# ielab/llm-rankers

Measured on AMD Instinct MI355X. Metric: passages/sec (pointwise yes_no reranking, flan-t5-large shape), higher is better.
Workload: dtype f16 (MFMA inputs), f32 accumulate + residual stream

## Files before the change

llm-rankers_amd/csrc/rk_engine.hip:

```cpp
#include <hip/hip_runtime.h>
#include <dlfcn.h>
#include <rccl/rccl.h>

#include <algorithm>
#include <cmath>
#include <cstdarg>
#include <cstdio>
#include <cstdlib>
#include <cstring>
#include <map>
#include <atomic>
#include <string>
#include <vector>

#include "../../include/rk_engine.h"
#include "attention.h"
#include "attention_d128.h"
#include "decoder_kernels.h"
#include "gemm.h"
#include "gemv_rows.h"
#include "llama_kernels.h"
#include "llama_kernels_hd64.h"
#include "misc_kernels.h"

// ... 50 lines not shown
template <class T>
struct Grown {
  T* p = nullptr; size_t cap = 0;
  Grown() = default;
  Grown(const Grown&) = delete;
  Grown& operator=(const Grown&) = delete;
  ~Grown() { if (p) hipFree(p); }
  int reserve(rk_engine* e, size_t n, int* gen = nullptr);
};

enum DecBuf { IX_DEC_IDS, IX_OUT_IDS, IX_LAST_ROWS, IX_N_CACHED, IX_ROW_LABEL = IX_N_CACHED, IX_ROW_OFF, IX_OUT_IDX, IX_ROW_SEQ, IX_TREE_KEYS, IX_TREE_POS, IX_COUNT };
struct DecIndex {
  struct Src { DecBuf b; const std::vector<int>& v; };
  int* d[IX_COUNT] = {nullptr};
  int* pin = nullptr;
  static constexpr int PIN_INTS = 8192;
  int put(rk_engine* e, hipStream_t st, DecBuf b, const int* src, int n);
  int write(rk_engine* e, hipStream_t st, std::initializer_list<Src> srcs);
  int tree(rk_engine* e, hipStream_t st, std::vector<int>& sig, std::initializer_list<Src> srcs);
 private:
  std::vector<int> held[IX_N_CACHED], tree_sig;
  unsigned long epoch = 0, tree_epoch = ~0ul;
};

}

#define RK_SLOTS 2

struct Slot {
  hipStream_t se = nullptr, sd = nullptr;
  NormStream enc;
  half_t *qkv = nullptr, *ctx = nullptr, *ffh = nullptr, *enc_out = nullptr;
  int* d_tokens = nullptr; int* d_seq_off = nullptr;
  int n_seq = 0, T = 0, maxL = 0, minL = 0; bool staged = false; int last_floats = 0;
  half_t* cross_kv = nullptr;
  DecIndex idx; int* d_argmax = nullptr;
  NormStream dec;
  half_t *dqkv = nullptr, *dctx = nullptr, *dq = nullptr, *dffh = nullptr, *dlast = nullptr;
  float* dssq_few[2] = {nullptr, nullptr};
  half_t *xqk = nullptr, *xctx = nullptr;
  float *xpart = nullptr, *xstat = nullptr; bool have_cross_kv = false;
  float* d_scores = nullptr; float* h_scores = nullptr;
  hipEvent_t ev_enc = nullptr, ev_dec = nullptr; bool dec_pending = false;
};

struct rk_engine {
  rk_model_desc d{};
  int dev = 0;
  std::string err;
  bool finalized = false;
  int inner = 0;
  std::map<std::string, HostTensor> host;
  std::vector<void*> allocs;
  half_t *emb = nullptr, *lm_head = nullptr, *cross_kv_w = nullptr;
  std::vector<EncLayerW> enc;
  std::vector<DecLayerW> dec;
  float *enc_final_ln = nullptr, *dec_final_ln = nullptr, *lut_enc = nullptr, *lut_dec = nullptr;
  Grown<float> logits;
  Grown<float> amax_val; Grown<int> amax_idx; int amax_gen = 0;
  Grown<half_t> kv_cache; int kv_gen = 0;
  Grown<int> gen_buf; int* gen_pin = nullptr; hipEvent_t ev_gen[2] = {nullptr, nullptr};
  size_t scores_cap = 0;
  Slot slots[RK_SLOTS];
  struct Options {
    int glds = 1, skinny = 0x3F, overlap = 1, gemm_variant = 0, attn_short = 5, xattn_direct = 1, attn_heads_per_wg = 0, attn_ko = 0,
        gemm_persistent = 1, fold_norm = 1, s64_stages = 0, dec_fold_norm = 1, greedy_spec = 160, consumer_stats = 1, xattn_mfma = 1,
        dec_ffn_tiled = 1, gemm_split = 1, dec_fuse = 1, dec_fuse_rows = 0, dec_attn_seq = 1, attn_long = 1, attn_long_nw = 0,
        llama_attn_dma = 1, attn_long_xcd = 1, llama_attn_nw = 0, dec_graph = 1, gemm_sk = 1, dec_cross_mfma = 1, dec_gemv = 1, dec_gemv_rows = 4,
        dec_cached_attn = 1, llama_dec_r = 0;
  } opt;
  float* attn_trace = nullptr;
  int n_cu = 256;
  struct SkWs { hipStream_t st = nullptr; float* slabs = nullptr; int* cnt = nullptr; };
  SkWs sk_ws[2 * RK_SLOTS];
  hipEvent_t t0 = nullptr, t1 = nullptr, t_tmp = nullptr;
  bool prof_on = false;
  std::vector<ProfRec> prof_recs; size_t prof_used = 0;
  double prof_flops[PC_COUNT] = {0}, prof_bytes[PC_COUNT] = {0}; int64_t prof_n[PC_COUNT] = {0};
  int family = 0; rk_llama_desc ld{};
  float rope_factor = 0.f, rope_low = 1.f, rope_high = 4.f; int rope_orig = 0;
  bool qkv_bias = false;
  int window = 0;
  std::vector<LlamaLayerW> ll; float *l_final_ln = nullptr, *rope_cos = nullptr, *rope_sin = nullptr; int* d_pos = nullptr;
  Grown<half_t> lkv; Grown<float> lpart; Grown<int> lints; int lkv_gen = 0;
  struct LlamaStep { NormStream stream; half_t *qkv = nullptr, *ctx = nullptr, *ffh = nullptr; } lg;
  struct LlamaSession {
    bool open = false; int n_slots = 0, max_len = 0, cap = 0, seen = 0;
    std::vector<int> busy, told, len, max_new, col, done;
  } ls;
  struct GraphEntry { int seen = 0; bool failed = false; hipGraphExec_t exec = nullptr; };
  std::map<std::vector<int>, GraphEntry> graphs; int opt_epoch = 0;
  ncclComm_t comm = nullptr; int comm_rank = 0, comm_world = 1;
  float* d_gather[RK_SLOTS] = {nullptr}; float* h_gather[RK_SLOTS] = {nullptr}; size_t gather_cap = 0;
  hipEvent_t ev_gather[RK_SLOTS] = {nullptr}; bool gather_pending[RK_SLOTS] = {false}; int gather_n[RK_SLOTS] = {0};
  float *d_gsend = nullptr, *d_gall = nullptr, *h_gall = nullptr, *h_gstage = nullptr;
  hipEvent_t ev_gall = nullptr, ev_append = nullptr; bool gall_pending = false, append_foreign = false; int gall_n = 0;
};

namespace {

int fail(rk_engine* e, int code, const char* fmt, ...) {
  char buf[1024];
// ... 831 lines not shown
  p.cgrid = dim3(n_heads, rows);
  p.window = e->window;
  return p;
}

void launch_llama_dec_attn(rk_engine* e, hipStream_t st, const LlamaDecAttnPlan& p, LlamaDecAttnArgs a, int rows) {
  a.nch = p.nch; a.window = p.window;
  Bracket br(e, st, PC_DEC_ATTN, 4.0 * rows * (double)a.P * a.n_heads * p.hd, 2.0 * rows * (double)a.P * a.n_kv * p.hd * 2.0);
  with_width(p.hd, [&](auto W) {
    constexpr int D = decltype(W)::value;
    auto go = [&](auto rc) {
      constexpr int R = decltype(rc)::value;
      if constexpr (R == 7 && D != 128) abort();
      else if (p.window > 0) {
        if (a.bias) hipLaunchKernelGGL((attn_dec_cached_win_kernel<D, R, true>), p.grid, dim3(256), 0, st, a);
        else hipLaunchKernelGGL((attn_dec_cached_win_kernel<D, R, false>), p.grid, dim3(256), 0, st, a);
      }
      else if (a.bias) hipLaunchKernelGGL((attn_dec_cached_kernel<D, R, true>), p.grid, dim3(256), 0, st, a);
      else hipLaunchKernelGGL((attn_dec_cached_kernel<D, R, false>), p.grid, dim3(256), 0, st, a);
    };
    using std::integral_constant;
    switch (p.R) {
      case 8: go(integral_constant<int, 8>{}); break;
      case 7: go(integral_constant<int, 7>{}); break;
      case 4: go(integral_constant<int, 4>{}); break;
      case 2: go(integral_constant<int, 2>{}); break;
      default: go(integral_constant<int, 1>{}); break;
    }
    if (p.window > 0) hipLaunchKernelGGL(attn_dec_combine_win_kernel<D>, p.cgrid, dim3(D), 0, st, a);
    else hipLaunchKernelGGL(attn_dec_combine_kernel<D>, p.cgrid, dim3(D), 0, st, a);
  });
}

int run_encoder(rk_engine* e, Slot& sl, bool need_cross_kv) {
  const rk_model_desc& d = e->d;
  hipStream_t st = enc_stream(e, sl);
  const int T = sl.T, I = e->inner, dm = d.d_model, F = d.d_ff;
  const bool own = e->opt.consumer_stats != 0;
  int rc = RK_OK;
  NormStream ns = sl.enc;
  const EncAttnPlan ap = plan_enc_attn(e, sl.n_seq, sl.maxL, sl.minL, d.n_heads);
  ns.begin(e, st, sl.d_tokens, T, e->opt.fold_norm != 0);
  for (int l = 0; l < d.n_enc_layers; ++l) {
    const EncLayerW& w = e->enc[l];
    const bool last = l + 1 == d.n_enc_layers;
    RC(gemm(e, st, ns.consumer(e, st, w.ln0, Gemm(PC_ENC_GEMM_QKV, EPI_STORE_F16, ns.x(), dm, ns.fold ? w.qkv_f : w.qkv, dm, sl.qkv, 3 * I, T, 3 * I, dm), own)));
    launch_enc_attn(e, st, EncAttnCall{sl.qkv, sl.ctx, sl.d_seq_off, e->lut_enc, 3 * I, I, I, d.n_heads, sl.n_seq, sl.maxL, sl.T}, ap);
    RC(ns.producer(e, st, Gemm(PC_ENC_GEMM_O, EPI_RESID_F32, sl.ctx, I, w.o, I, ns.hidden, dm, T, dm, I)));
    RC(gemm(e, st, ns.consumer(e, st, w.ln1, Gemm(PC_ENC_GEMM_FFN_IN, d.gated_gelu ? EPI_GEGLU_F16 : EPI_RELU_F16, ns.x(), dm, ns.fold ? w.ffn_in_f : w.ffn_in, dm,
                                                 sl.ffh, F, T, d.gated_gelu ? 2 * F : F, dm), own)));
    RC(ns.producer(e, st, Gemm(PC_ENC_GEMM_FFN_OUT, EPI_RESID_F32, sl.ffh, F, w.ffn_out, F, ns.hidden, dm, T, dm, F), !last));
  }
  rmsnorm(e, st, ns.hidden, e->enc_final_ln, sl.enc_out, nullptr, T);
  if (need_cross_kv)
    RC(gemm(e, st, Gemm(PC_GEMM_CROSS_KV, EPI_STORE_F16, sl.enc_out, dm, e->cross_kv_w, dm, sl.cross_kv, 2 * I, T, d.n_dec_layers * 2 * I, dm)
                       .split(2 * I, (long)d.max_tokens * 2 * I)));
  sl.have_cross_kv = need_cross_kv;
  HIPCHK(e, hipGetLastError());
  return RK_OK;
}

struct DecRows {
  int rows; const int* keys; const int* pos; const int* seq;
  const int* row_off; int seq0, n_seq; bool cross_kv; const int* ids;
  bool tree() const { return keys != nullptr; }
};
struct DecCache { half_t* kv; int P; const int* pos; const int* tree_keys; int* tree_pos; };
void launch_dec_cached_step(const rk_engine* e, hipStream_t st, const AttnCachedArgs& ca, int B, int H, const int* tree_keys, int* tree_pos) {
  if (e->opt.dec_cached_attn) {
    hipLaunchKernelGGL(attn_dec_cached_kernel, dim3(H, B), dim3(256), attn_dec_lds(ca.P), st, ca);
  } else {
    hipLaunchKernelGGL(kv_append_kernel, dim3(B), dim3(256), 0, st, ca, tree_pos);
    hipLaunchKernelGGL(attn_dec_kernel, dim3(1, H, B), dim3(256), attn_dec_lds(ca.P), st,
                       AttnDecArgs{ca.qkv, ca.ldqkv, ca.cache, ca.cache + ca.inner, 2 * ca.inner, nullptr, ca.ctx, ca.ldctx, ca.bias_lut, ca.P, 1, ca.P,
                                   tree_keys, tree_pos});
  }
}
int run_decoder(rk_engine* e, Slot& sl, int Ld, const DecRows* rows = nullptr, const DecCache* cache = nullptr) {
  const rk_model_desc& d = e->d;
  hipStream_t st = dec_stream(e, sl);
  const bool tree = rows && rows->tree(), ragged = rows && !rows->tree();
  const int B = ragged ? rows->n_seq : sl.n_seq, M = rows ? rows->rows : B * Ld, I = e->inner, dm = d.d_model, F = d.d_ff;
  const bool have_kv = ragged ? rows->cross_kv : sl.have_cross_kv;
  const int* seq_off = sl.d_seq_off + (ragged ? rows->seq0 : 0);
  const DecLenClass lc = dec_len_class(e, Ld);
  if (tree && (have_kv || lc.one)) return fail(e, RK_ERR_STATE, "the tree form needs the query-side cross-attention and L_d >= 2");
  if (ragged && have_kv && !sl.have_cross_kv) return fail(e, RK_ERR_STATE, "the ragged pass needs the K / V the encoder did not materialise");
  if (cache && (rows || have_kv || Ld != 1)) return fail(e, RK_ERR_STATE, "the incremental pass needs the query-side cross-attention and one row per sequence");
  if (wide_heads(e) && (!lc.one || rows || cache || have_kv || e->opt.dec_fuse == 2))
    return refuse_wide(e, "run_decoder", "this pass would launch a 64-wide kernel");
  const bool ws = lc.stream;
  const bool dfold = ws && e->opt.dec_fold_norm && (e->opt.skinny & 0x3F) == 0x3F;
  const bool fuse_asked = e->opt.dec_fuse == 2 || (e->opt.dec_fuse == 1 && lc.one);
  const bool few = dfold && e->opt.dec_gemv && !lc.one && M <= e->opt.dec_gemv_rows && !fuse_asked &&
                   gemv_fits(M, dm) && gemv_fits(M, I) && gemv_fits(M, F);
  const GemmFamily fam = few ? GEMM_GEMV : (ws ? GEMM_STREAM : GEMM_TILED);
  int rc = RK_OK;
  NormStream ns = sl.dec;
  if (few) { ns.ssq[0] = sl.dssq_few[0]; ns.ssq[1] = sl.dssq_few[1]; }
  auto normed = [&](const float* ln, Gemm c) { return ns.consumer(e, st, ln, c.on(fam), true); };
  auto resid = [&](Gemm c, bool stats = true) { return ns.producer(e, st, c.on(fam), stats); };
  ns.begin(e, st, ragged && rows->ids ? rows->ids : sl.idx.d[IX_DEC_IDS], M, dfold);
  const DecAttnPlan self_plan = plan_dec_attn(e, false, B, Ld, Ld, d.n_heads, tree ? rows->rows : 0);
  const DecAttnPlan cross_plan = plan_dec_attn(e, true, B, Ld, sl.maxL, d.n_heads, 0);
  for (int l = 0; l < d.n_dec_layers; ++l) {
    const DecLayerW& w = e->dec[l];
    if (!cache && lc.one) {
      RC(resid(normed(w.ln0, Gemm(PC_DEC_GEMM, EPI_RESID_F32, ns.x(), dm, dfold ? w.ov_f : w.ov, dm, ns.hidden, dm, M, dm, dm))));
    } else {
      RC(gemm(e, st, normed(w.ln0, Gemm(PC_DEC_GEMM, EPI_STORE_F16, ns.x(), dm, dfold ? w.qkv_f : w.qkv, dm, sl.dqkv, 3 * I, M, 3 * I, dm))));
      if (cache) {
        const AttnCachedArgs ca{sl.dqkv, 3 * I, cache->kv + (size_t)l * B * cache->P * 2 * I, cache->P, I, cache->pos, sl.dctx, I, e->lut_dec};
        Bracket br(e, st, PC_DEC_ATTN, 4.0 * B * (double)cache->P * I, (double)B * cache->P * 2 * I * 2.0);
        launch_dec_cached_step(e, st, ca, B, d.n_heads, cache->tree_keys, cache->tree_pos);
      } else {
        launch_dec_attn(e, st, self_plan, AttnDecArgs{sl.dqkv, 3 * I, sl.dqkv + I, sl.dqkv + 2 * I, 3 * I, nullptr, sl.dctx, I, e->lut_dec, Ld, 1, Ld,
                                                      tree ? rows->keys : nullptr, tree ? rows->pos : nullptr, 0, ragged ? rows->row_off : nullptr},
                        4.0 * M * Ld * I, 0);
      }
      RC(resid(Gemm(PC_DEC_GEMM, EPI_RESID_F32, sl.dctx, I, w.o, I, ns.hidden, dm, M, dm, I)));
    }
    const Gemm cq = normed(w.ln1, Gemm(PC_DEC_GEMM, EPI_STORE_F16, ns.x(), dm, dfold ? w.cq_f : w.cq, dm, sl.dq, I, M, I, dm));
    if (!have_kv) {
      RC(run_xattn_chain(e, st, XAttnChain{cq.A, cq.lda, cq.W, w.ckT, e->cross_kv_w + ((size_t)l * 2 * I + I) * dm, cq.fold, cq.family,
                                           sl.enc_out, sl.d_seq_off, rows ? rows->seq : nullptr, Ld, 0, sl.dq, sl.xqk, sl.xpart, sl.xstat, sl.xctx,
                                           sl.dctx, I, M, d.n_heads, dm, sl.maxL, sl.T, fuse_asked, head_width(e)}));
    } else {
      RC(gemm(e, st, cq));
      const half_t* kv = sl.cross_kv + (size_t)l * d.max_tokens * 2 * I;
      launch_dec_attn(e, st, cross_plan, AttnDecArgs{sl.dq, I, kv, kv + I, 2 * I, seq_off, sl.dctx, I, nullptr, Ld, 0, sl.maxL, nullptr, nullptr, 0,
                                                       ragged ? rows->row_off : nullptr},
                      4.0 * Ld * (double)sl.T * I, (double)sl.T * 2 * I * 2.0);
    }
    RC(resid(Gemm(PC_DEC_GEMM, EPI_RESID_F32, sl.dctx, I, w.co, I, ns.hidden, dm, M, dm, I)));
    {
      const bool tiled_in = dfold && e->opt.dec_ffn_tiled && lc.one;
      RC(gemm(e, st, ns.consumer(e, st, w.ln2, Gemm(PC_DEC_GEMM, d.gated_gelu ? EPI_GEGLU_F16 : EPI_RELU_F16, ns.x(), dm, dfold ? w.ffn_in_f : w.ffn_in, dm,
                                                   sl.dffh, F, M, d.gated_gelu ? 2 * F : F, dm).on(tiled_in ? GEMM_TILED : fam), true)));
    }
    RC(resid(Gemm(PC_DEC_GEMM, EPI_RESID_F32, sl.dffh, F, w.ffn_out, F, ns.hidden, dm, M, dm, F), l + 1 < d.n_dec_layers));
  }
  HIPCHK(e, hipGetLastError());
  return RK_OK;
}

int encoder_then_handoff_kv(rk_engine* e, Slot& sl, bool need_cross_kv) {
  hipStream_t se = enc_stream(e, sl), sd = dec_stream(e, sl);
  if (need_cross_kv && !sl.cross_kv) return refuse_wide(e, "encoder", "the materialised cross-attention K / V are not allocated");
  if (sl.dec_pending && sd != se) HIPCHK(e, hipStreamWaitEvent(se, sl.ev_dec, 0));
  int rc = run_encoder(e, sl, need_cross_kv);
  if (rc) return rc;
  if (sd != se) {
    HIPCHK(e, hipEventRecord(sl.ev_enc, se));
    HIPCHK(e, hipStreamWaitEvent(sd, sl.ev_enc, 0));
  }
  return RK_OK;
}

int encoder_then_handoff(rk_engine* e, Slot& sl, int max_ld, bool query_side = false) {
  return encoder_then_handoff_kv(e, sl, !query_side && !use_xattn_direct(e, sl, max_ld));
}

int mark_decoder_done(rk_engine* e, Slot& sl) {
  HIPCHK(e, hipEventRecord(sl.ev_dec, dec_stream(e, sl)));
  sl.dec_pending = true;
  return RK_OK;
}

int sync_all(rk_engine* e) {
  for (Slot& sl : e->slots) {
    HIPCHK(e, hipStreamSynchronize(sl.se));
    HIPCHK(e, hipStreamSynchronize(sl.sd));
  }
  return RK_OK;
}

int finish_blocking(rk_engine* e, Slot& sl) {
  int rc = mark_decoder_done(e, sl);
  if (rc || (rc = sync_all(e))) return rc;
  sl.dec_pending = false;
  return RK_OK;
}

template <class T>
int Grown<T>::reserve(rk_engine* e, size_t n, int* gen) {
  if (n <= cap) return RK_OK;
  int rc = sync_all(e);
  if (rc) return rc;
// ... 44 lines not shown
int put_dec_ids_shared(rk_engine* e, Slot& sl, const int32_t* prefix, int Ld) {
  std::vector<int> ids((size_t)sl.n_seq * Ld);
  for (int b = 0; b < sl.n_seq; ++b) memcpy(&ids[(size_t)b * Ld], prefix, Ld * sizeof(int));
  return sl.idx.put(e, dec_stream(e, sl), IX_DEC_IDS, ids.data(), (int)ids.size());
}

void shift_right(const int32_t* labels, int n, std::vector<int>* out) {
  for (int t = 0; t < n; ++t) out->push_back(t ? labels[t - 1] : 0);
}

int check_greedy_args(rk_engine* e, const int32_t* dec_prefix, int dec_len, int max_new) {
  if (!dec_prefix || dec_len <= 0 || max_new <= 0 || dec_len + max_new - 1 > e->d.max_dec_len)
    return fail(e, RK_ERR_CAPACITY, "dec_len %d + max_new %d exceeds max_dec_len %d", dec_len, max_new, e->d.max_dec_len);
  return RK_OK;
}

int read_scores_blocking(rk_engine* e, Slot& sl, hipStream_t st, size_t n, float* out) {
  HIPCHK(e, hipMemcpyAsync(sl.h_scores, sl.d_scores, n * sizeof(float), hipMemcpyDeviceToHost, st));
  if (e->family == 0) { const int rc = finish_blocking(e, sl); if (rc) return rc; }
  else HIPCHK(e, hipStreamSynchronize(st));
  HIPCHK(e, hipGetLastError());
  memcpy(out, sl.h_scores, n * sizeof(float));
  return RK_OK;
}

int stage_slot(rk_engine* e, int slot, const int32_t* tokens, const int32_t* seq_offsets, int n_seq) {
  if (slot < 0 || slot >= RK_SLOTS) return fail(e, RK_ERR_INVALID, "slot %d out of range", slot);
  if (e->family != 0) return fail(e, RK_ERR_STATE, "T5 entry point called on a Llama engine (use rk_llama_*)");
  int rc = set_device(e);
  if (rc) return rc;
  Slot& sl = e->slots[slot];
  sl.staged = false;
  if ((rc = check_batch(e, &sl, tokens, seq_offsets, n_seq))) return rc;
  if (sl.dec_pending) { HIPCHK(e, hipEventSynchronize(sl.ev_dec)); sl.dec_pending = false; }
  HIPCHK(e, hipStreamSynchronize(enc_stream(e, sl)));
  HIPCHK(e, hipMemcpy(sl.d_tokens, tokens, (size_t)sl.T * sizeof(int), hipMemcpyHostToDevice));
  HIPCHK(e, hipMemcpy(sl.d_seq_off, seq_offsets, (size_t)(n_seq + 1) * sizeof(int), hipMemcpyHostToDevice));
  sl.staged = true;
  return RK_OK;
}

enum GraphKind { GK_T5_SCORE, GK_T5_GREEDY_STEP, GK_T5_GREEDY2, GK_T5_GENERATE_STEP, GK_LLAMA_STEP, GK_T5_COMPARE, GK_LLAMA_SESSION_STEP };
template <class F>
int run_graphed(rk_engine* e, hipStream_t st, std::vector<int> key, F&& body) {
  key.push_back(e->opt_epoch);
  if (!e->opt.dec_graph || e->prof_on) return body();
  auto& g = e->graphs[key];
  if (g.exec) { HIPCHK(e, hipGraphLaunch(g.exec, st)); return RK_OK; }
  if (g.failed || g.seen++ == 0) return body();
  if (e->graphs.size() > 256) {
    for (auto& kv : e->graphs) if (kv.second.exec && &kv.second != &g) { hipGraphExecDestroy(kv.second.exec); kv.second.exec = nullptr; kv.second.seen = 0; }
  }
  hipGraph_t graph = nullptr;
  if (hipStreamBeginCapture(st, hipStreamCaptureModeThreadLocal) != hipSuccess) { (void)hipGetLastError(); g.failed = true; return body(); }
  const int rc = body();
  const hipError_t ec = hipStreamEndCapture(st, &graph);
  if (rc != RK_OK || ec != hipSuccess || !graph) {
    (void)hipGetLastError();
    if (graph) hipGraphDestroy(graph);
    g.failed = true;
    return rc != RK_OK ? rc : body();
  }
  const hipError_t ei = hipGraphInstantiate(&g.exec, graph, nullptr, nullptr, 0);
  hipGraphDestroy(graph);
  if (ei != hipSuccess || !g.exec) { (void)hipGetLastError(); g.exec = nullptr; g.failed = true; return body(); }
  HIPCHK(e, hipGraphLaunch(g.exec, st));
  return RK_OK;
}

int ensure_decode_ring(rk_engine* e) {
// ... 210 lines not shown
  const rk_model_desc& d = *desc;
  if (d.d_kv != 64 && d.d_kv != 128)
    return fail(nullptr, RK_ERR_INVALID, "d_kv=%d unsupported: the gfx950 attention kernels are built for d_kv=64 and, for one decoder position, d_kv=128", d.d_kv);
  if (d.d_model % 64 || (d.n_heads * d.d_kv) % 64 || d.d_ff % 64 || d.vocab % 4)
    return fail(nullptr, RK_ERR_INVALID, "d_model, n_heads*d_kv, d_ff must be multiples of 64 and vocab of 4");
  if (d.d_model > 4096)
    return fail(nullptr, RK_ERR_INVALID, "d_model=%d unsupported: rmsnorm_kernel holds a row of at most 4096 columns in registers (d_model <= 4096)", d.d_model);
  if (d.max_distance > RK_LUT_R || d.n_buckets < 4 || d.n_buckets > 256)
    return fail(nullptr, RK_ERR_INVALID, "relative attention config unsupported (max_distance<=%d)", RK_LUT_R);
  if (d.max_tokens <= 0 || d.max_seqs <= 0 || d.max_dec_len <= 0 || d.n_enc_layers <= 0 || d.n_dec_layers <= 0)
    return fail(nullptr, RK_ERR_INVALID, "capacities and layer counts must be positive");
  if ((long)d.max_seqs * d.max_dec_len > 8192 * 8) return fail(nullptr, RK_ERR_INVALID, "max_seqs*max_dec_len too large");
  int n_dev = 0;
  if (hipGetDeviceCount(&n_dev) != hipSuccess || n_dev <= 0)
    return fail(nullptr, RK_ERR_NO_DEVICE, "no HIP device visible: this engine has no CPU path");
  if (device_ordinal < 0 || device_ordinal >= n_dev)
    return fail(nullptr, RK_ERR_NO_DEVICE, "device ordinal %d out of range (%d devices)", device_ordinal, n_dev);
  hipDeviceProp_t prop;
  if (hipGetDeviceProperties(&prop, device_ordinal) != hipSuccess)
    return fail(nullptr, RK_ERR_HIP, "hipGetDeviceProperties failed");
  if (strncmp(prop.gcnArchName, "gfx950", 6) != 0)
    return fail(nullptr, RK_ERR_NO_DEVICE, "device %d is %s; kernels are built for gfx950 (MI355X) only", device_ordinal, prop.gcnArchName);
  rk_engine* e = new rk_engine();
  e->d = d; e->dev = device_ordinal; e->n_cu = prop.multiProcessorCount > 0 ? prop.multiProcessorCount : 256; e->inner = d.n_heads * d.d_kv;
  int prio_lo = 0, prio_hi = 0;
  bool ok = hipSetDevice(device_ordinal) == hipSuccess;
  ok = ok && hipDeviceGetStreamPriorityRange(&prio_lo, &prio_hi) == hipSuccess;
  for (int i = 0; ok && i < RK_SLOTS; ++i)
    ok = hipStreamCreateWithPriority(&e->slots[i].se, hipStreamNonBlocking, prio_lo) == hipSuccess &&
         hipStreamCreateWithPriority(&e->slots[i].sd, hipStreamNonBlocking, prio_hi) == hipSuccess;
  ok = ok && hipEventCreate(&e->t0) == hipSuccess && hipEventCreate(&e->t1) == hipSuccess &&
       hipEventCreateWithFlags(&e->t_tmp, hipEventDisableTiming) == hipSuccess;
  for (int i = 0; ok && i < RK_SLOTS; ++i)
    ok = hipEventCreateWithFlags(&e->slots[i].ev_enc, hipEventDisableTiming) == hipSuccess &&
         hipEventCreateWithFlags(&e->slots[i].ev_dec, hipEventDisableTiming) == hipSuccess;
  for (int i = 0; ok && i < 2 * RK_SLOTS; ++i) {
    rk_engine::SkWs& w = e->sk_ws[i];
    w.st = (i & 1) ? e->slots[i >> 1].sd : e->slots[i >> 1].se;
    ok = hipMalloc((void**)&w.slabs, (size_t)KSPLIT_MAX_SLABS * 65536 * sizeof(float)) == hipSuccess &&
         hipMalloc((void**)&w.cnt, KSPLIT_MAX_SLABS * sizeof(int)) == hipSuccess &&
         hipMemset(w.cnt, 0, KSPLIT_MAX_SLABS * sizeof(int)) == hipSuccess;
  }
  if (!ok) {
    for (auto& w : e->sk_ws) { if (w.slabs) hipFree(w.slabs); if (w.cnt) hipFree(w.cnt); }
    delete e;
    return fail(nullptr, RK_ERR_HIP, "stream/event/workspace creation failed");
  }
  *out = e;
  return RK_OK;
}

void rk_engine_destroy(rk_engine* e) {
  if (!e) return;
  hipSetDevice(e->dev);
  for (auto& sl : e->slots) {
    if (sl.se) hipStreamSynchronize(sl.se);
    if (sl.sd) hipStreamSynchronize(sl.sd);
  }
  comm_release(e);
  for (auto& kv : e->graphs) if (kv.second.exec) hipGraphExecDestroy(kv.second.exec);
  e->graphs.clear();
  for (void* p : e->allocs) hipFree(p);
  if (e->gen_pin) hipHostFree(e->gen_pin);
  for (hipEvent_t ev : e->ev_gen) if (ev) hipEventDestroy(ev);
  for (auto& w : e->sk_ws) { if (w.slabs) hipFree(w.slabs); if (w.cnt) hipFree(w.cnt); }
  for (auto& sl : e->slots) {
    if (sl.h_scores) hipHostFree(sl.h_scores);
    if (sl.idx.pin) hipHostFree(sl.idx.pin);
    if (sl.ev_enc) hipEventDestroy(sl.ev_enc);
    if (sl.ev_dec) hipEventDestroy(sl.ev_dec);
  }
  for (auto& r : e->prof_recs) { hipEventDestroy(r.a); hipEventDestroy(r.b); }
  if (e->t0) hipEventDestroy(e->t0);
  if (e->t1) hipEventDestroy(e->t1);
  if (e->t_tmp) hipEventDestroy(e->t_tmp);
  for (auto& sl : e->slots) {
    if (sl.se) hipStreamDestroy(sl.se);
    if (sl.sd) hipStreamDestroy(sl.sd);
  }
  delete e;
}

int rk_engine_load_tensor(rk_engine* e, const char* hf_name, const void* data, int dtype, const int64_t* shape, int ndim) {
  if (!e || !hf_name || !data || !shape) return fail(e, RK_ERR_INVALID, "null argument");
  if (e->finalized) return fail(e, RK_ERR_STATE, "engine already finalized");
  if (ndim < 1 || ndim > 2) return RK_OK;
  std::string name(hf_name);
  if (name == "encoder.embed_tokens.weight" || name == "decoder.embed_tokens.weight") return RK_OK;
  size_t n = 1;
  for (int i = 0; i < ndim; ++i) n *= (size_t)shape[i];
  HostTensor t;
  t.shape.assign(shape, shape + ndim);
  const bool keep_f32 = ndim == 1 || name.find("relative_attention_bias") != std::string::npos;
  auto get = [&](size_t i) -> float {
    switch (dtype) {
      case RK_F32: return ((const float*)data)[i];
      case RK_F16: return (float)((const half_t*)data)[i];
      case RK_BF16: { uint32_t u = (uint32_t)((const uint16_t*)data)[i] << 16; float f; memcpy(&f, &u, 4); return f; }
      default: return 0.f;
    }
  };
  if (dtype < RK_F32 || dtype > RK_BF16) return fail(e, RK_ERR_INVALID, "unknown dtype %d", dtype);
// ... 125 lines not shown
  RC(up_h(&e->cross_kv_w, ckv));
  {
    half_t* d_vT = nullptr; float* d_ov32 = nullptr;
    RC(dalloc(e, &d_vT, (size_t)dm * I)); RC(dalloc(e, &d_ov32, (size_t)dm * dm));
    std::vector<half_t> vT((size_t)dm * I), ov16((size_t)dm * dm);
    std::vector<float> ov32((size_t)dm * dm);
    for (int l = 0; l < d.n_dec_layers; ++l) {
      const std::string p = "decoder.block." + std::to_string(l) + ".layer.0.SelfAttention.";
      const auto& wv = H(p + "v.weight");
      for (int j = 0; j < I; ++j)
        for (int k = 0; k < dm; ++k) vT[(size_t)k * I + j] = wv[(size_t)j * dm + k];
      HIPCHK(e, hipMemcpy(d_vT, vT.data(), vT.size() * 2, hipMemcpyHostToDevice));
      RC(gemm(e, e->slots[0].se, Gemm(PC_OTHER, EPI_STORE_F32, e->dec[l].o, I, d_vT, I, d_ov32, dm, dm, dm, I)));
      HIPCHK(e, hipStreamSynchronize(e->slots[0].se));
      HIPCHK(e, hipMemcpy(ov32.data(), d_ov32, ov32.size() * 4, hipMemcpyDeviceToHost));
      for (size_t i = 0; i < ov32.size(); ++i) ov16[i] = (half_t)ov32[i];
      RC(up_h(&e->dec[l].ov, ov16));
      const auto& ln0 = Fv("decoder.block." + std::to_string(l) + ".layer.0.layer_norm.weight");
      for (size_t i = 0; i < ov32.size(); ++i) ov16[i] = (half_t)(ov32[i] * ln0[i % dm]);
      RC(up_h(&e->dec[l].ov_f, ov16));
    }
    HIPCHK(e, hipGetLastError());
  }
  e->host.clear();

  const size_t Tc = d.max_tokens, Bc = d.max_seqs, Mc = (size_t)d.max_seqs * d.max_dec_len;
  e->scores_cap = Bc * 64;
  if (2 * e->scores_cap < 7 * Bc) return fail(e, RK_ERR_CAPACITY, "score buffer of %zu floats cannot hold a compare of %zu sequences", e->scores_cap, Bc);
  for (Slot& sl : e->slots) {
    RC(dalloc(e, &sl.enc.hidden, Tc * dm)); RC(dalloc(e, &sl.enc.xn, Tc * dm)); RC(dalloc(e, &sl.qkv, Tc * 3 * I));
    RC(dalloc(e, &sl.ctx, Tc * I)); RC(dalloc(e, &sl.ffh, Tc * F)); RC(dalloc(e, &sl.enc_out, Tc * dm));
    RC(dalloc(e, &sl.enc.xraw[0], Tc * dm)); RC(dalloc(e, &sl.enc.ssq[0], Tc * ((dm + 63) / 64))); RC(dalloc(e, &sl.enc.factors, Tc + 512));
    HIPCHK(e, hipMemset(sl.enc.factors, 0, (Tc + 512) * sizeof(float)));
    RC(dalloc(e, &sl.d_tokens, Tc)); RC(dalloc(e, &sl.d_seq_off, Bc + 1));
    if (!wide_heads(e)) RC(dalloc(e, &sl.cross_kv, (size_t)d.n_dec_layers * Tc * 2 * I));
    RC(dalloc(e, &sl.idx.d[IX_DEC_IDS], Mc)); RC(dalloc(e, &sl.idx.d[IX_LAST_ROWS], Bc)); RC(dalloc(e, &sl.idx.d[IX_OUT_IDS], 8192));
    RC(dalloc(e, &sl.idx.d[IX_ROW_LABEL], Mc)); RC(dalloc(e, &sl.idx.d[IX_ROW_OFF], 2 * Bc + 1)); RC(dalloc(e, &sl.idx.d[IX_OUT_IDX], Bc)); RC(dalloc(e, &sl.d_argmax, Bc));
    RC(dalloc(e, &sl.idx.d[IX_ROW_SEQ], Mc)); RC(dalloc(e, &sl.idx.d[IX_TREE_KEYS], Mc * (size_t)d.max_dec_len)); RC(dalloc(e, &sl.idx.d[IX_TREE_POS], Mc));
    RC(dalloc(e, &sl.dec.hidden, Mc * dm)); RC(dalloc(e, &sl.dec.xn, Mc * dm)); RC(dalloc(e, &sl.dqkv, Mc * 3 * I));
    RC(dalloc(e, &sl.dctx, Mc * I)); RC(dalloc(e, &sl.dq, Mc * I)); RC(dalloc(e, &sl.dffh, Mc * F));
    RC(dalloc(e, &sl.dlast, Bc * dm));
    for (int i = 0; i < 2; ++i) { RC(dalloc(e, &sl.dec.xraw[i], Mc * dm)); RC(dalloc(e, &sl.dec.ssq[i], Mc * ((dm + 31) / 32))); RC(dalloc(e, &sl.dssq_few[i], (size_t)GEMV_MAX_ROWS * e->n_cu)); }
    RC(dalloc(e, &sl.dec.factors, Mc));
    RC(dalloc(e, &sl.xqk, (size_t)XA_MAX_ROWS * d.n_heads * dm)); RC(dalloc(e, &sl.xctx, (size_t)XA_MAX_ROWS * d.n_heads * dm));
    RC(dalloc(e, &sl.xpart, (size_t)XA_MAX_CHUNKS * d.n_heads * dm)); RC(dalloc(e, &sl.xstat, (size_t)XA_MAX_CHUNKS * d.n_heads * 2));
    RC(dalloc(e, &sl.d_scores, e->scores_cap));
    HIPCHK(e, hipHostMalloc((void**)&sl.h_scores, e->scores_cap * sizeof(float), hipHostMallocDefault));
    HIPCHK(e, hipHostMalloc((void**)&sl.idx.pin, IX_N_CACHED * DecIndex::PIN_INTS * sizeof(int), hipHostMallocDefault));
  }
  const int dec_smem_max = (int)attn_dec_lds(std::max(d.max_tokens, d.max_dec_len));
  (void)hipFuncSetAttribute((const void*)attn_dec_kernel, hipFuncAttributeMaxDynamicSharedMemorySize, std::min(dec_smem_max, 160 * 1024));
  (void)hipFuncSetAttribute((const void*)attn_dec_seq_kernel, hipFuncAttributeMaxDynamicSharedMemorySize, 160 * 1024);
#define GEMM_ATTR(EPI)                                                                                              \
  (void)hipFuncSetAttribute((const void*)gemm_f16_kernel<EPI, true>, hipFuncAttributeMaxDynamicSharedMemorySize, GEMM_LDS_BYTES); \
  (void)hipFuncSetAttribute((const void*)gemm_f16_kernel<EPI, false>, hipFuncAttributeMaxDynamicSharedMemorySize, GEMM_LDS_BYTES);
  GEMM_ATTR(EPI_STORE_F16) GEMM_ATTR(EPI_RESID_F32) GEMM_ATTR(EPI_GEGLU_F16) GEMM_ATTR(EPI_RELU_F16) GEMM_ATTR(EPI_STORE_F32) GEMM_ATTR(EPI_SWIGLU_F16)
#undef GEMM_ATTR
  (void)hipGetLastError();
  HIPCHK(e, hipDeviceSynchronize());
  e->finalized = true;
  return RK_OK;
}

int rk_t5_stage_slot(rk_engine* e, int slot, const int32_t* tokens, const int32_t* seq_offsets, int n_seq) {
  if (!e) return RK_ERR_INVALID;
  return stage_slot(e, slot, tokens, seq_offsets, n_seq);
}
// ... 1036 lines not shown

namespace {
struct OptionDesc { const char* key; int rk_engine::Options::*field; int lo, hi; const char* allowed; const char* what; };
const OptionDesc kOptions[] = {
  {"dec_graph", &rk_engine::Options::dec_graph, 0, 1, nullptr, "decoder chains replayed as HIP graphs (1) or launched eagerly (0)"},
  {"gemm_glds", &rk_engine::Options::glds, 0, 1, nullptr, "128x128 GEMM staging by LDS-DMA (1) or through registers (0); same bits"},
  {"gemm_skinny", &rk_engine::Options::skinny, 0, 0x3F, nullptr, "bit per epilogue kind: few-row GEMMs on the weight-streaming kernel (1 = all)"},
  {"dec_ffn_tiled", &rk_engine::Options::dec_ffn_tiled, 0, 1, nullptr, "one-position decoder: FFN-in on the tiled kernels (1) or the weight-streaming kernel (0)"},
  {"gemm_persistent", &rk_engine::Options::gemm_persistent, 0, 1024, nullptr, "ping-pong GEMM: 1 = one workgroup per CU walks the tiles, 0 = one per tile, n > 1 = n workgroups"},
  {"gemm_s64_stages", &rk_engine::Options::s64_stages, 0, 4, "0,2,3,4", "LDS stages of the 64x64 GEMM (0 = from the tile count); same bits"},
  {"consumer_stats", &rk_engine::Options::consumer_stats, 0, 1, nullptr, "encoder row factors formed by the non-persistent consumer GEMMs themselves (1) or always by rowscale_kernel (0); same bits"},
  {"greedy_spec", &rk_engine::Options::greedy_spec, 0, 65536, nullptr, "rk_t5_greedy2: most decoder rows of a speculative pass; 0 = never speculate; same tokens"},
  {"dec_fold_norm", &rk_engine::Options::dec_fold_norm, 0, 1, nullptr, "decoder RMSNorms folded into the weight-streaming GEMMs (1) or separate kernels (0)"},
  {"fold_norm", &rk_engine::Options::fold_norm, 0, 1, nullptr, "encoder RMSNorm folded into the GEMMs (1) or separate kernels (0)"},
  {"xattn_mfma", &rk_engine::Options::xattn_mfma, 0, 1, nullptr, "query-side cross-attention: weighted sums on the matrix cores (1) or the VALU form (0)"},
  {"attn_heads_per_wg", &rk_engine::Options::attn_heads_per_wg, 0, 4096, nullptr, "short-sequence attention: (sequence, head) items per wave group, 0 = dealt evenly; same bits"},
  {"xattn_direct", &rk_engine::Options::xattn_direct, 0, 1, nullptr, "decoder prefixes <= 16: query-side cross-attention (1) or materialised K / V (0)"},
  {"attn_short", &rk_engine::Options::attn_short, 0, 6, "0,5,6", "sequences <= 192 keys: DMA kernel with two (5) / one (6) wave group per workgroup, or the tiled kernel (0); same bits"},
  {"gemm_variant", &rk_engine::Options::gemm_variant, 0, 120, nullptr, "tile variant: 0 auto, 1..6 see choose_variant; measurement builds: 80+ / 100+ knock-outs"},
  {"dec_fuse_rows", &rk_engine::Options::dec_fuse_rows, 0, 32, nullptr, "rows per workgroup of dec_cross_qk_kernel (0 = auto); same bits"},
  {"dec_fuse", &rk_engine::Options::dec_fuse, 0, 2, nullptr, "few-row decoder: projections around the query-side cross-attention fused at one position (1), always (2), never (0)"},
  {"llama_attn_nw", &rk_engine::Options::llama_attn_nw, 0, 8, "0,4,8", "waves per workgroup of the Llama LDS-DMA attention kernel (0 = default 4); same bits"},
  {"llama_attn_dma", &rk_engine::Options::llama_attn_dma, 0, 1, nullptr, "Llama causal attention: LDS-DMA kernel (1) or the register-staged first kernel (0); differ within fp16 noise"},
  {"attn_long_xcd", &rk_engine::Options::attn_long_xcd, 0, 1, nullptr, "long-sequence attention: workgroups of a (sequence, head) pair on one XCD (1) or dealt over all eight (0); same bits"},
  {"attn_long_nw", &rk_engine::Options::attn_long_nw, 0, 12, "0,3,4,6,12", "waves per workgroup of the long-sequence attention kernel (0 = default 4); same bits"},
  {"attn_long", &rk_engine::Options::attn_long, 0, 1, nullptr, "sequences > 192 keys: the chunked LDS-DMA kernel (1) or the tiled kernel (0)"},
  {"dec_gemv", &rk_engine::Options::dec_gemv, 0, 1, nullptr, "decoder pass of at most 16 rows at >= 2 positions (one setwise compare): plain projections on the wave-per-column GEMV kernel (1) or the weight-streaming MFMA kernel (0); differ within fp32 summation-order noise"},
  {"dec_gemv_rows", &rk_engine::Options::dec_gemv_rows, 1, GEMV_MAX_ROWS, nullptr, "largest row count of a decoder pass that takes the few-row GEMV family (default 4 = the measured cross-over; the kernel takes up to 16)"},
  {"dec_cross_mfma", &rk_engine::Options::dec_cross_mfma, 0, 1, nullptr, "long decoder prefixes (qlm), cross-attention over the materialised K / V: matrix-core kernel for sequences <= 192 keys (1) or the staged fma-chain kernels (0); differ within fp16 noise"},
  {"dec_attn_seq", &rk_engine::Options::dec_attn_seq, 0, 1, nullptr, "decoder attention at several positions: one workgroup per (head, sequence) (1) or per query row (0); same bits"},
  {"gemm_sk", &rk_engine::Options::gemm_sk, 0, 2, nullptr, "ping-pong GEMM, fp32 residual projections with few tiles and a long K: K split over two workgroups (1: choose_ksplit), never (0), wherever it fits (2: tests)"},
  {"dec_cached_attn", &rk_engine::Options::dec_cached_attn, 0, 1, nullptr, "rk_t5_generate's self-attention: attn_dec_cached_kernel (1) or the cache append + attn_dec_kernel's tree form (0); same bits"},
  {"llama_dec_r", &rk_engine::Options::llama_dec_r, 0, 2, nullptr, "rk_llama_generate's attention: query heads per workgroup by plan_llama_dec_attn's rule (0), one (1), or, where a kv head has 7, all seven (2: measurement and tests; every cached K / V byte read once per step); same bits"},
  {"gemm_split", &rk_engine::Options::gemm_split, 0, 1, nullptr, "rows beyond the ping-pong kernel's last whole round on a fill-in tile variant (1) or one launch (0); same bits"},
#ifdef RK_MEASURE
  {"attn_ko", &rk_engine::Options::attn_ko, 0, 1 << 20, nullptr, "timing-only knock-outs of the attention kernels (measurement builds)"},
#endif
};
bool option_value_ok(const OptionDesc& o, int value) {
  if (value < o.lo || value > o.hi) return false;
  if (!o.allowed) return true;
  for (const char* p = o.allowed; *p;) {
    if (atoi(p) == value) return true;
    while (*p && *p != ',') ++p;
    if (*p == ',') ++p;
  }
  return false;
}
}

extern "C" {

int rk_engine_set_option(rk_engine* e, const char* key, int value) {
  if (!e || !key) return RK_ERR_INVALID;
  if (!strcmp(key, "overlap")) {
    if (value < 0 || value > 1) return fail(e, RK_ERR_INVALID, "option overlap: 0..1");
    if (set_device(e) || sync_all(e)) return RK_ERR_HIP;
    for (Slot& sl : e->slots) sl.dec_pending = false;
    e->opt.overlap = value;
    e->opt_epoch++;
    return RK_OK;
  }
#ifdef RK_MEASURE
  if (!strcmp(key, "attn_trace")) {
    if (value && !e->attn_trace) { if (hipMalloc(&e->attn_trace, 12 * 16 * 16 * sizeof(float)) != hipSuccess) return RK_ERR_HIP; hipMemset(e->attn_trace, 0, 12 * 16 * 16 * sizeof(float)); }
    if (!value && e->attn_trace) { hipFree(e->attn_trace); e->attn_trace = nullptr; }
// ... 828 lines not shown
```

Measured before the change: 7589.

## Double-buffer staged tokens so encoder layers overlap previous slot decoder

Token and sequence-offset staging buffers are double-buffered per slot, with one encoder-done event per generation. Staging now waits only for the encoder that last read the buffer, instead of synchronizing the decoder and the whole encoder stream. The encoder waits for the previous decoder only before its final norm and cross-KV projection, so its layers can run alongside that decoder. A separate decoder copy of the sequence offsets is copied in on device, and an option can serialize encoder chains across slots. This adds buffers and event bookkeeping, plus a risk of ordering bugs.

After: 7776, median of 6. +2.5%, better.

```diff
diff --git a/llm-rankers_amd/csrc/rk_engine.hip b/llm-rankers_amd/csrc/rk_engine.hip
--- a/llm-rankers_amd/csrc/rk_engine.hip
+++ b/llm-rankers_amd/csrc/rk_engine.hip
@@ -106,6 +106,9 @@
   NormStream enc;
   half_t *qkv = nullptr, *ctx = nullptr, *ffh = nullptr, *enc_out = nullptr;
   int* d_tokens = nullptr; int* d_seq_off = nullptr;
+  int* dec_seq_off = nullptr;
+  int *stg_tokens[2] = {nullptr, nullptr}, *stg_seq_off[2] = {nullptr, nullptr};
+  int gen = 0; bool gen_launched = false; unsigned stage_no = 0, off_of = 0;
   int n_seq = 0, T = 0, maxL = 0, minL = 0; bool staged = false; int last_floats = 0;
   half_t* cross_kv = nullptr;
   DecIndex idx; int* d_argmax = nullptr;
@@ -115,7 +118,7 @@
   half_t *xqk = nullptr, *xctx = nullptr;
   float *xpart = nullptr, *xstat = nullptr; bool have_cross_kv = false;
   float* d_scores = nullptr; float* h_scores = nullptr;
-  hipEvent_t ev_enc = nullptr, ev_dec = nullptr; bool dec_pending = false;
+  hipEvent_t ev_enc[2] = {nullptr, nullptr}, ev_dec = nullptr; int enc_gen = -1; bool dec_pending = false;
 };
 
 struct rk_engine {
@@ -141,7 +144,7 @@
         gemm_persistent = 1, fold_norm = 1, s64_stages = 0, dec_fold_norm = 1, greedy_spec = 160, consumer_stats = 1, xattn_mfma = 1,
         dec_ffn_tiled = 1, gemm_split = 1, dec_fuse = 1, dec_fuse_rows = 0, dec_attn_seq = 1, attn_long = 1, attn_long_nw = 0,
         llama_attn_dma = 1, attn_long_xcd = 1, llama_attn_nw = 0, dec_graph = 1, gemm_sk = 1, dec_cross_mfma = 1, dec_gemv = 1, dec_gemv_rows = 4,
-        dec_cached_attn = 1, llama_dec_r = 0;
+        dec_cached_attn = 1, llama_dec_r = 0, enc_serial = 0;
   } opt;
   float* attn_trace = nullptr;
   int n_cu = 256;
@@ -1039,6 +1042,12 @@
   });
 }
 
+int wait_prev_decoder(rk_engine* e, Slot& sl) {
+  hipStream_t se = enc_stream(e, sl);
+  if (sl.dec_pending && dec_stream(e, sl) != se) HIPCHK(e, hipStreamWaitEvent(se, sl.ev_dec, 0));
+  return RK_OK;
+}
+
 int run_encoder(rk_engine* e, Slot& sl, bool need_cross_kv) {
   const rk_model_desc& d = e->d;
   hipStream_t st = enc_stream(e, sl);
@@ -1047,16 +1056,22 @@
   int rc = RK_OK;
   NormStream ns = sl.enc;
   const EncAttnPlan ap = plan_enc_attn(e, sl.n_seq, sl.maxL, sl.minL, d.n_heads);
-  ns.begin(e, st, sl.d_tokens, T, e->opt.fold_norm != 0);
+  const int* seq_off = sl.stg_seq_off[sl.gen];
+  ns.begin(e, st, sl.stg_tokens[sl.gen], T, e->opt.fold_norm != 0);
   for (int l = 0; l < d.n_enc_layers; ++l) {
     const EncLayerW& w = e->enc[l];
     const bool last = l + 1 == d.n_enc_layers;
     RC(gemm(e, st, ns.consumer(e, st, w.ln0, Gemm(PC_ENC_GEMM_QKV, EPI_STORE_F16, ns.x(), dm, ns.fold ? w.qkv_f : w.qkv, dm, sl.qkv, 3 * I, T, 3 * I, dm), own)));
-    launch_enc_attn(e, st, EncAttnCall{sl.qkv, sl.ctx, sl.d_seq_off, e->lut_enc, 3 * I, I, I, d.n_heads, sl.n_seq, sl.maxL, sl.T}, ap);
+    launch_enc_attn(e, st, EncAttnCall{sl.qkv, sl.ctx, seq_off, e->lut_enc, 3 * I, I, I, d.n_heads, sl.n_seq, sl.maxL, sl.T}, ap);
     RC(ns.producer(e, st, Gemm(PC_ENC_GEMM_O, EPI_RESID_F32, sl.ctx, I, w.o, I, ns.hidden, dm, T, dm, I)));
     RC(gemm(e, st, ns.consumer(e, st, w.ln1, Gemm(PC_ENC_GEMM_FFN_IN, d.gated_gelu ? EPI_GEGLU_F16 : EPI_RELU_F16, ns.x(), dm, ns.fold ? w.ffn_in_f : w.ffn_in, dm,
                                                  sl.ffh, F, T, d.gated_gelu ? 2 * F : F, dm), own)));
     RC(ns.producer(e, st, Gemm(PC_ENC_GEMM_FFN_OUT, EPI_RESID_F32, sl.ffh, F, w.ffn_out, F, ns.hidden, dm, T, dm, F), !last));
+  }
+  RC(wait_prev_decoder(e, sl));
+  if (sl.off_of != sl.stage_no) {
+    HIPCHK(e, hipMemcpyAsync(sl.dec_seq_off, seq_off, (size_t)(sl.n_seq + 1) * sizeof(int), hipMemcpyDeviceToDevice, st));
+    sl.off_of = sl.stage_no;
   }
   rmsnorm(e, st, ns.hidden, e->enc_final_ln, sl.enc_out, nullptr, T);
   if (need_cross_kv)
@@ -1089,7 +1104,7 @@
   const bool tree = rows && rows->tree(), ragged = rows && !rows->tree();
   const int B = ragged ? rows->n_seq : sl.n_seq, M = rows ? rows->rows : B * Ld, I = e->inner, dm = d.d_model, F = d.d_ff;
   const bool have_kv = ragged ? rows->cross_kv : sl.have_cross_kv;
-  const int* seq_off = sl.d_seq_off + (ragged ? rows->seq0 : 0);
+  const int* seq_off = sl.dec_seq_off + (ragged ? rows->seq0 : 0);
   const DecLenClass lc = dec_len_class(e, Ld);
   if (tree && (have_kv || lc.one)) return fail(e, RK_ERR_STATE, "the tree form needs the query-side cross-attention and L_d >= 2");
   if (ragged && have_kv && !sl.have_cross_kv) return fail(e, RK_ERR_STATE, "the ragged pass needs the K / V the encoder did not materialise");
@@ -1130,7 +1145,7 @@
     const Gemm cq = normed(w.ln1, Gemm(PC_DEC_GEMM, EPI_STORE_F16, ns.x(), dm, dfold ? w.cq_f : w.cq, dm, sl.dq, I, M, I, dm));
     if (!have_kv) {
       RC(run_xattn_chain(e, st, XAttnChain{cq.A, cq.lda, cq.W, w.ckT, e->cross_kv_w + ((size_t)l * 2 * I + I) * dm, cq.fold, cq.family,
-                                           sl.enc_out, sl.d_seq_off, rows ? rows->seq : nullptr, Ld, 0, sl.dq, sl.xqk, sl.xpart, sl.xstat, sl.xctx,
+                                           sl.enc_out, sl.dec_seq_off, rows ? rows->seq : nullptr, Ld, 0, sl.dq, sl.xqk, sl.xpart, sl.xstat, sl.xctx,
                                            sl.dctx, I, M, d.n_heads, dm, sl.maxL, sl.T, fuse_asked, head_width(e)}));
     } else {
       RC(gemm(e, st, cq));
@@ -1154,13 +1169,15 @@
 int encoder_then_handoff_kv(rk_engine* e, Slot& sl, bool need_cross_kv) {
   hipStream_t se = enc_stream(e, sl), sd = dec_stream(e, sl);
   if (need_cross_kv && !sl.cross_kv) return refuse_wide(e, "encoder", "the materialised cross-attention K / V are not allocated");
-  if (sl.dec_pending && sd != se) HIPCHK(e, hipStreamWaitEvent(se, sl.ev_dec, 0));
-  int rc = run_encoder(e, sl, need_cross_kv);
+  static_assert(RK_SLOTS == 2, "the other slot");
+  const Slot& other = e->slots[(&sl - e->slots) ^ 1];
+  if (e->opt.enc_serial && sd != se && other.enc_gen >= 0) HIPCHK(e, hipStreamWaitEvent(se, other.ev_enc[other.enc_gen], 0));
+  sl.gen_launched = true;
+  const int rc = run_encoder(e, sl, need_cross_kv);
+  HIPCHK(e, hipEventRecord(sl.ev_enc[sl.gen], se));
+  sl.enc_gen = sl.gen;
   if (rc) return rc;
-  if (sd != se) {
-    HIPCHK(e, hipEventRecord(sl.ev_enc, se));
-    HIPCHK(e, hipStreamWaitEvent(sd, sl.ev_enc, 0));
-  }
+  if (sd != se) HIPCHK(e, hipStreamWaitEvent(sd, sl.ev_enc[sl.gen], 0));
   return RK_OK;
 }
 
@@ -1271,10 +1288,11 @@
   Slot& sl = e->slots[slot];
   sl.staged = false;
   if ((rc = check_batch(e, &sl, tokens, seq_offsets, n_seq))) return rc;
-  if (sl.dec_pending) { HIPCHK(e, hipEventSynchronize(sl.ev_dec)); sl.dec_pending = false; }
-  HIPCHK(e, hipStreamSynchronize(enc_stream(e, sl)));
-  HIPCHK(e, hipMemcpy(sl.d_tokens, tokens, (size_t)sl.T * sizeof(int), hipMemcpyHostToDevice));
-  HIPCHK(e, hipMemcpy(sl.d_seq_off, seq_offsets, (size_t)(n_seq + 1) * sizeof(int), hipMemcpyHostToDevice));
+  const int g = sl.gen_launched ? sl.gen ^ 1 : sl.gen;
+  HIPCHK(e, hipEventSynchronize(sl.ev_enc[g]));
+  HIPCHK(e, hipMemcpy(sl.stg_tokens[g], tokens, (size_t)sl.T * sizeof(int), hipMemcpyHostToDevice));
+  HIPCHK(e, hipMemcpy(sl.stg_seq_off[g], seq_offsets, (size_t)(n_seq + 1) * sizeof(int), hipMemcpyHostToDevice));
+  sl.gen = g; sl.gen_launched = false; ++sl.stage_no;
   sl.staged = true;
   return RK_OK;
 }
@@ -1551,7 +1569,8 @@
   ok = ok && hipEventCreate(&e->t0) == hipSuccess && hipEventCreate(&e->t1) == hipSuccess &&
        hipEventCreateWithFlags(&e->t_tmp, hipEventDisableTiming) == hipSuccess;
   for (int i = 0; ok && i < RK_SLOTS; ++i)
-    ok = hipEventCreateWithFlags(&e->slots[i].ev_enc, hipEventDisableTiming) == hipSuccess &&
+    ok = hipEventCreateWithFlags(&e->slots[i].ev_enc[0], hipEventDisableTiming) == hipSuccess &&
+         hipEventCreateWithFlags(&e->slots[i].ev_enc[1], hipEventDisableTiming) == hipSuccess &&
          hipEventCreateWithFlags(&e->slots[i].ev_dec, hipEventDisableTiming) == hipSuccess;
   for (int i = 0; ok && i < 2 * RK_SLOTS; ++i) {
     rk_engine::SkWs& w = e->sk_ws[i];
@@ -1586,7 +1605,7 @@
   for (auto& sl : e->slots) {
     if (sl.h_scores) hipHostFree(sl.h_scores);
     if (sl.idx.pin) hipHostFree(sl.idx.pin);
-    if (sl.ev_enc) hipEventDestroy(sl.ev_enc);
+    for (hipEvent_t ev : sl.ev_enc) if (ev) hipEventDestroy(ev);
     if (sl.ev_dec) hipEventDestroy(sl.ev_dec);
   }
   for (auto& r : e->prof_recs) { hipEventDestroy(r.a); hipEventDestroy(r.b); }
@@ -1778,7 +1797,8 @@
     RC(dalloc(e, &sl.ctx, Tc * I)); RC(dalloc(e, &sl.ffh, Tc * F)); RC(dalloc(e, &sl.enc_out, Tc * dm));
     RC(dalloc(e, &sl.enc.xraw[0], Tc * dm)); RC(dalloc(e, &sl.enc.ssq[0], Tc * ((dm + 63) / 64))); RC(dalloc(e, &sl.enc.factors, Tc + 512));
     HIPCHK(e, hipMemset(sl.enc.factors, 0, (Tc + 512) * sizeof(float)));
-    RC(dalloc(e, &sl.d_tokens, Tc)); RC(dalloc(e, &sl.d_seq_off, Bc + 1));
+    for (int g = 0; g < 2; ++g) { RC(dalloc(e, &sl.stg_tokens[g], Tc)); RC(dalloc(e, &sl.stg_seq_off[g], Bc + 1)); }
+    RC(dalloc(e, &sl.dec_seq_off, Bc + 1));
     if (!wide_heads(e)) RC(dalloc(e, &sl.cross_kv, (size_t)d.n_dec_layers * Tc * 2 * I));
     RC(dalloc(e, &sl.idx.d[IX_DEC_IDS], Mc)); RC(dalloc(e, &sl.idx.d[IX_LAST_ROWS], Bc)); RC(dalloc(e, &sl.idx.d[IX_OUT_IDS], 8192));
     RC(dalloc(e, &sl.idx.d[IX_ROW_LABEL], Mc)); RC(dalloc(e, &sl.idx.d[IX_ROW_OFF], 2 * Bc + 1)); RC(dalloc(e, &sl.idx.d[IX_OUT_IDX], Bc)); RC(dalloc(e, &sl.d_argmax, Bc));
@@ -2881,6 +2901,7 @@
   {"gemm_sk", &rk_engine::Options::gemm_sk, 0, 2, nullptr, "ping-pong GEMM, fp32 residual projections with few tiles and a long K: K split over two workgroups (1: choose_ksplit), never (0), wherever it fits (2: tests)"},
   {"dec_cached_attn", &rk_engine::Options::dec_cached_attn, 0, 1, nullptr, "rk_t5_generate's self-attention: attn_dec_cached_kernel (1) or the cache append + attn_dec_kernel's tree form (0); same bits"},
   {"llama_dec_r", &rk_engine::Options::llama_dec_r, 0, 2, nullptr, "rk_llama_generate's attention: query heads per workgroup by plan_llama_dec_attn's rule (0), one (1), or, where a kv head has 7, all seven (2: measurement and tests; every cached K / V byte read once per step); same bits"},
+  {"enc_serial", &rk_engine::Options::enc_serial, 0, 1, nullptr, "two slots: an encoder chain starts behind the other slot's (1: one encoder at a time beside the decoder before it) or as soon as it is enqueued (0: two chains interleave); same bits"},
   {"gemm_split", &rk_engine::Options::gemm_split, 0, 1, nullptr, "rows beyond the ping-pong kernel's last whole round on a fill-in tile variant (1) or one launch (0); same bits"},
 #ifdef RK_MEASURE
   {"attn_ko", &rk_engine::Options::attn_ko, 0, 1 << 20, nullptr, "timing-only knock-outs of the attention kernels (measurement builds)"},
```
